# sephiroce/srf

Measured on AMD Instinct MI355X. Metric: acoustic frames/sec through SRF (123-d fbank, 3-iter DR) at 1/2/4/8 MI355X, higher is better.
Workload: dtype fp32; 1 GPU; wsj_c4: SRF L=6 PH=CH=16 DIM=32 LPAD=RPAD=2 DR iter=3, train step (fwd+bwd+allreduce+Adam); utterances_per_gpu=28, frames_per_utterance=800, global_batch=28, parallelism=dp1, launch=hipgraph (fwd+CTC+bwd)

## Files before the change

### srf_amd/csrc/cnnfe.hip

```cpp
#include <algorithm>
#include <cmath>
#include <cstdlib>

#include "srf_common.h"
#include "srf_reduce.h"
#include "srf_rng.h"
#include "../../include/srf.h"

namespace {

constexpr int C = 64;
constexpr float kBnEps = 1e-3f;
constexpr float kBnMomentum = 0.99f;

struct Dims {
  int B, T, Fin;
  int T1, F1, T2, F2;
  int pt1, pf1, pt2, pf2;
};

inline int same_out(int n) { return (n + 1) / 2; }
inline int same_pad_before(int n) {
  const int out = same_out(n);
  const int total = std::max((out - 1) * 2 + 3 - n, 0);
  return total / 2;
}

Dims make_dims(int B, int T, int Fin) {
  Dims d;
  d.B = B; d.T = T; d.Fin = Fin;
  d.T1 = same_out(T); d.F1 = same_out(Fin);
  d.T2 = same_out(d.T1); d.F2 = same_out(d.F1);
  d.pt1 = same_pad_before(T); d.pf1 = same_pad_before(Fin);
  d.pt2 = same_pad_before(d.T1); d.pf2 = same_pad_before(d.F1);
  return d;
}

__device__ __forceinline__ int ceil_div_len(int len, int div) { return (len + div - 1) / div; }

__device__ __forceinline__ void chan_merge(float& n, float& mean, float& m2, float nb, float meanb, float m2b) {
  if (nb == 0.f) return;
  const float nn = n + nb;
  const float delta = meanb - mean;
  mean += delta * (nb / nn);
  m2 += m2b + delta * delta * (n * nb / nn);
  n = nn;
}

constexpr int kPackW2Threads = 2 * C * 64;
__device__ __forceinline__ void pack_w2_f16_body(int idx, const float* __restrict__ ka, const float* __restrict__ kb,
                                                 _Float16* __restrict__ wp2, float* __restrict__ wsc);
__device__ __forceinline__ void pack_w2t_f16_body(int idx, const float* __restrict__ ka, const float* __restrict__ kb,
                                                  _Float16* __restrict__ wq2h, float* __restrict__ wdsc);
constexpr int kPackW2tF16Threads = C * 64;

constexpr int kRows1 = 4;

struct Tile1 {
  int b, t1_0, fpad;
};

__device__ __forceinline__ Tile1 stage_rows1(const float* __restrict__ feats, const Dims& d, float* win) {
  const int tiles_per_b = (d.T1 + kRows1 - 1) / kRows1;
  Tile1 tl;
  tl.b = blockIdx.x / tiles_per_b;
  tl.t1_0 = (blockIdx.x - tl.b * tiles_per_b) * kRows1;
  tl.fpad = d.Fin + 2;
  const int nrows = 2 * kRows1 + 1;
  const int t_base = 2 * tl.t1_0 - d.pt1;
  for (int k = threadIdx.x; k < nrows * tl.fpad; k += blockDim.x) {
    const int r = k / tl.fpad, col = k - r * tl.fpad;
    const int t = t_base + r, f = col - 1;
    const bool ok = t >= 0 && t < d.T && f >= 0 && f < d.Fin;
    const float v = feats[((size_t)tl.b * d.T + min(max(t, 0), d.T - 1)) * d.Fin + min(max(f, 0), d.Fin - 1)];
    win[k] = ok ? v : 0.f;
  }
  __syncthreads();
  return tl;
}

__device__ __forceinline__ void window9_lds(const float* win, const Tile1& tl, const Dims& d, int w, int f1,
                                            float (&x)[9]) {
#pragma unroll
  for (int dt = 0; dt < 3; ++dt)
#pragma unroll
    for (int df = 0; df < 3; ++df) x[dt * 3 + df] = win[(2 * w + dt) * tl.fpad + 2 * f1 - d.pf1 + df + 1];
}

__global__ __launch_bounds__(256) void conv1_fwd_kernel(
    const float* __restrict__ feats, const int* __restrict__ inp_len, Dims d, const float* __restrict__ ka,
    const float* __restrict__ ba, const float* __restrict__ kb, const float* __restrict__ bb, int training,
    float drop_p, unsigned long long seed, const unsigned long long* __restrict__ seed_src, float* __restrict__ y1, unsigned char* __restrict__ sel1,
    float* __restrict__ part, int nconv, const float* __restrict__ pk_a, const float* __restrict__ pk_b,
    _Float16* __restrict__ wp2, float* __restrict__ wsc, float* __restrict__ ymax) {
  if ((int)blockIdx.x >= nconv) {
    const int idx = (blockIdx.x - nconv) * blockDim.x + threadIdx.x;
    if (idx < kPackW2Threads) pack_w2_f16_body(idx, pk_a, pk_b, wp2, wsc);
    return;
  }
  seed = srf_step_seed(seed, seed_src);
  extern __shared__ __attribute__((aligned(16))) float win[];
  __shared__ float sh[3][kRows1][C];
  const int c = threadIdx.x & (C - 1);
  const int w = __builtin_amdgcn_readfirstlane(threadIdx.x >> 6);
  float wa[9], wb[9];
#pragma unroll
  for (int k = 0; k < 9; ++k) {
    wa[k] = ka[k * C + c];
    wb[k] = kb[k * C + c];
  }
  const float bia = ba[c], bib = bb[c];
  const float keep_scale = 1.f / (1.f - drop_p);
  const bool drop = training && drop_p > 0.f;
  const Tile1 tl = stage_rows1(feats, d, win);
  const int t1 = tl.t1_0 + w;
  float n = 0.f, s1 = 0.f, s2 = 0.f, ym = 0.f;
  const float K = 0.5f * (bia + bib);
  if (t1 < d.T1) {
    const bool live = t1 < ceil_div_len(inp_len[tl.b], 2);
    const int pbase = (tl.b * d.T1 + t1) * d.F1;
#pragma unroll 2
    for (int f1 = 0; f1 < d.F1; ++f1) {
      float x[9];
      window9_lds(win, tl, d, w, f1, x);
      float a = bia, bv = bib;
#pragma unroll
      for (int k = 0; k < 9; ++k) {
        a += x[k] * wa[k];
        bv += x[k] * wb[k];
      }
      const int o = (pbase + f1) * C + c;
      if (drop) {
        bool ka, kb;
        srf_keep2(seed, kStreamConv0a, o, drop_p, ka, kb);
        a *= ka ? keep_scale : 0.f;
        bv *= kb ? keep_scale : 0.f;
      }
      const bool sl = a >= bv;
      const float y = live ? (sl ? a : bv) : 0.f;
      y1[o] = y;
      sel1[o] = sl ? 1 : 0;
      ym = fmaxf(ym, fabsf(y));
      n += 1.f;
      s1 += y - K;
      s2 += (y - K) * (y - K);
    }
  }
  float mean = n > 0.f ? K + s1 / n : 0.f;
  float m2 = n > 0.f ? fmaxf(s2 - s1 * s1 / n, 0.f) : 0.f;
  sh[0][w][c] = n; sh[1][w][c] = mean; sh[2][w][c] = m2;
#pragma unroll
  for (int o = 32; o >= 1; o >>= 1) ym = fmaxf(ym, __shfl_xor(ym, o, 64));
  __shared__ float smax[kRows1];
  if (c == 0) smax[w] = ym;
  __syncthreads();
  if (w == 0) {
    if (c == 0) {
      float m = smax[0];
      for (int r = 1; r < kRows1; ++r) m = fmaxf(m, smax[r]);
      ymax[blockIdx.x] = m;
    }
    for (int r = 1; r < kRows1; ++r) chan_merge(n, mean, m2, sh[0][r][c], sh[1][r][c], sh[2][r][c]);
    part[((size_t)blockIdx.x * 3 + 0) * C + c] = n;
    part[((size_t)blockIdx.x * 3 + 1) * C + c] = mean;
    part[((size_t)blockIdx.x * 3 + 2) * C + c] = m2;
  }
}

__global__ __launch_bounds__(256) void bn_merge_kernel(const float* __restrict__ part, int nparts, int per,
                                                       float* __restrict__ out) {
  __shared__ float sh[3][4][C];
  const int c = threadIdx.x & (C - 1), r = threadIdx.x >> 6;
  const int k0 = blockIdx.x * per, k1 = min(nparts, k0 + per);
  float n = 0.f, mu = 0.f, m2 = 0.f;
  for (int k = k0 + r; k < k1; k += 4)
    chan_merge(n, mu, m2, part[((size_t)k * 3 + 0) * C + c], part[((size_t)k * 3 + 1) * C + c],
               part[((size_t)k * 3 + 2) * C + c]);
  sh[0][r][c] = n; sh[1][r][c] = mu; sh[2][r][c] = m2;
  __syncthreads();
  if (r != 0) return;
  for (int q = 1; q < 4; ++q) chan_merge(n, mu, m2, sh[0][q][c], sh[1][q][c], sh[2][q][c]);
  out[((size_t)blockIdx.x * 3 + 0) * C + c] = n;
  out[((size_t)blockIdx.x * 3 + 1) * C + c] = mu;
  out[((size_t)blockIdx.x * 3 + 2) * C + c] = m2;
}

__global__ __launch_bounds__(1024) void bn_finalize_kernel(const float* __restrict__ part, int nparts,
                                                           const float* __restrict__ gamma,
                                                           const float* __restrict__ beta,
                                                           float* __restrict__ mmean, float* __restrict__ mvar,
                                                           int training, float* __restrict__ stats,
                                                           const float* __restrict__ ymax, int nymax) {
  __shared__ float sh[3][16][C];
  __shared__ float ysh[16], ab[2][C];
  const int c = threadIdx.x & (C - 1), r = threadIdx.x >> 6;
  if (ymax != nullptr) {
    float m = 0.f;
    for (int k = threadIdx.x; k < nymax; k += 1024) m = fmaxf(m, ymax[k]);
#pragma unroll
    for (int o = 32; o >= 1; o >>= 1) m = fmaxf(m, __shfl_xor(m, o, 64));
    if (c == 0) ysh[r] = m;
  }
  float n = 0.f, mu = 0.f, m2 = 0.f;
  if (training)
#pragma unroll 8
    for (int k = r; k < nparts; k += 16)
      chan_merge(n, mu, m2, part[((size_t)k * 3 + 0) * C + c], part[((size_t)k * 3 + 1) * C + c],
                 part[((size_t)k * 3 + 2) * C + c]);
  sh[0][r][c] = n; sh[1][r][c] = mu; sh[2][r][c] = m2;
  __syncthreads();
  if (r == 0) {
    float mean, var;
    if (training) {
      for (int q = 1; q < 16; ++q) chan_merge(n, mu, m2, sh[0][q][c], sh[1][q][c], sh[2][q][c]);
      mean = mu;
      var = m2 / n;
      mmean[c] = mmean[c] * kBnMomentum + mean * (1.f - kBnMomentum);
      mvar[c] = mvar[c] * kBnMomentum + (n > 1.f ? var * n / (n - 1.f) : var) * (1.f - kBnMomentum);
    } else {
      mean = mmean[c];
      var = mvar[c];
    }
    const float rstd = 1.f / sqrtf(var + kBnEps);
    const float scale = gamma[c] * rstd;
    const float shift = beta[c] - mean * scale;
    stats[0 * C + c] = mean;
    stats[1 * C + c] = rstd;
    stats[2 * C + c] = scale;
    stats[3 * C + c] = shift;
    ab[0][c] = fabsf(scale);
    ab[1][c] = fabsf(shift);
  }
  if (ymax == nullptr) return;
  __syncthreads();
  if (threadIdx.x == 0) {
    float y = ysh[0], sa = 0.f, sb = 0.f;
    for (int q = 1; q < 16; ++q) y = fmaxf(y, ysh[q]);
    for (int q = 0; q < C; ++q) {
      sa = fmaxf(sa, ab[0][q]);
      sb = fmaxf(sb, ab[1][q]);
    }
    const int e = srf_split_exp(sa * y + sb);
    stats[4 * C + 0] = srf_exp2i(e);
    stats[4 * C + 1] = srf_exp2i(-e);
  }
}


__device__ __forceinline__ void split2h8(const float (&v)[8], h8& p1, h8& p2, float sc = 1.f) {
#pragma unroll
  for (int k = 0; k < 8; ++k) {
    _Float16 h1, h2;
    srf_split2h(v[k] * sc, h1, h2);
    p1[k] = h1;
    p2[k] = h2;
  }
}
__device__ __forceinline__ f16v mfma3h(const h8& a1, const h8& a2, const h8& b1, const h8& b2, f16v c) {
  c = mfma32h(a2, b1, c);
  c = mfma32h(a1, b2, c);
  return mfma32h(a1, b1, c);
}

__device__ __forceinline__ void pack_w2_f16_body(int idx, const float* __restrict__ ka, const float* __restrict__ kb,
                                                 _Float16* __restrict__ wp2, float* __restrict__ wsc) {
  const int n = idx >> 6, cin = idx & 63;
  const float* k = n < C ? ka : kb;
  const int co = n % C;
  float v[9], m = 0.f;
#pragma unroll
  for (int tap = 0; tap < 9; ++tap) {
    v[tap] = k[((size_t)tap * C + cin) * C + co];
    m = fmaxf(m, fabsf(v[tap]));
  }
#pragma unroll
  for (int o = 32; o >= 1; o >>= 1) m = fmaxf(m, __shfl_xor(m, o, 64));
  const int e = srf_split_exp(m);
  const float sc = srf_exp2i(e);
  const size_t plane = (size_t)9 * 2 * C * C;
#pragma unroll
  for (int tap = 0; tap < 9; ++tap) {
    _Float16 h1, h2;
    srf_split2h(v[tap] * sc, h1, h2);
    const size_t o = ((size_t)tap * 2 * C + n) * C + cin;
    wp2[o] = h1;
    wp2[plane + o] = h2;
  }
  if (cin == 0) wsc[n] = srf_exp2i(-e);
}

constexpr int kC2BStride = 24;
constexpr int kC2Waves = 4;
constexpr int kC2Px = 32 * kC2Waves;
constexpr int kC2BLoads = 2 * 2 * C * 2 / (64 * kC2Waves);

__global__ __launch_bounds__(64 * kC2Waves) __attribute__((amdgpu_waves_per_eu(2))) void conv2_fwd32_kernel(
    const float* __restrict__ y1, const float* __restrict__ stats1, const int* __restrict__ inp_len, Dims d,
    const _Float16* __restrict__ wp2, const float* __restrict__ wsc, const float* __restrict__ ba,
    const float* __restrict__ bb, int training, float drop_p, unsigned long long seed,
    const unsigned long long* __restrict__ seed_src, float* __restrict__ y2, unsigned char* __restrict__ sel2,
    float* __restrict__ part) {
  seed = srf_step_seed(seed, seed_src);
  __shared__ __attribute__((aligned(16))) _Float16 Bs[2][2][2 * C * kC2BStride];
  __shared__ __attribute__((aligned(16))) float ss[2][C];
  __shared__ float red[3][kC2Waves][2 * 32];
  const int tid = threadIdx.x;
  const int lane = tid & 63, wv = tid >> 6;
  const int r = lane & 31, h = lane >> 5;
  const int P2 = d.B * d.T2 * d.F2;
  const int p0 = blockIdx.x * kC2Px;
  const size_t plane = (size_t)9 * 2 * C * C;
  if (tid < 2 * C) ss[tid >> 6][tid & 63] = stats1[(2 + (tid >> 6)) * C + (tid & 63)] * stats1[4 * C];

  const int pa = p0 + 32 * wv + r;
  const bool alive = pa < P2;
  const int pc = min(pa, P2 - 1);
  const int af2 = pc % d.F2, at2 = (pc / d.F2) % d.T2, ab = pc / (d.F2 * d.T2);
  const int alen1 = ceil_div_len(inp_len[ab], 2);

  auto load_b = [&](int kk, h8 (&bv)[kC2BLoads]) {
    const int tap = kk >> 2, kb = kk & 3;
#pragma unroll
    for (int q = 0; q < kC2BLoads; ++q) {
      const int idx = q * 64 * kC2Waves + tid;
      const int pl = idx >> 8, rem = idx & 255, n = rem >> 1, half = rem & 1;
      bv[q] = *reinterpret_cast<const h8*>(wp2 + pl * plane + ((size_t)tap * 2 * C + n) * C + 16 * kb + 8 * half);
    }
  };
  auto store_b = [&](int buf, const h8 (&bv)[kC2BLoads]) {
#pragma unroll
    for (int q = 0; q < kC2BLoads; ++q) {
      const int idx = q * 64 * kC2Waves + tid;
      const int pl = idx >> 8, rem = idx & 255, n = rem >> 1, half = rem & 1;
      *reinterpret_cast<h8*>(&Bs[buf][pl][n * kC2BStride + 8 * half]) = bv[q];
    }
  };
  auto load_a = [&](int kk, f4 (&av)[2], bool& ok) {
    const int tap = kk >> 2, kb = kk & 3;
    const int dt = tap / 3, df = tap - dt * 3;
    const int t1 = 2 * at2 - d.pt2 + dt, f1 = 2 * af2 - d.pf2 + df;
    ok = alive && t1 >= 0 && t1 < d.T1 && f1 >= 0 && f1 < d.F1 && t1 < alen1;
    const int t1c = min(max(t1, 0), d.T1 - 1), f1c = min(max(f1, 0), d.F1 - 1);
    const float* src = y1 + (((size_t)ab * d.T1 + t1c) * d.F1 + f1c) * C + 16 * kb + 8 * h;
    av[0] = *reinterpret_cast<const f4*>(src);
    av[1] = *reinterpret_cast<const f4*>(src + 4);
  };

  f16v acc[4];
#pragma unroll
  for (int nt = 0; nt < 4; ++nt) acc[nt] = f16v{};
  auto compute = [&](int kk, int buf, const f4 (&av)[2], bool aok) {
    h8 a1, a2;
    {
      const int c0 = 16 * (kk & 3) + 8 * h;
      float v[8];
#pragma unroll
      for (int q = 0; q < 8; ++q) {
        const float x = q < 4 ? av[0][q] : av[1][q - 4];
        v[q] = aok ? x * ss[0][c0 + q] + ss[1][c0 + q] : 0.f;
      }
      split2h8(v, a1, a2);
    }
#pragma unroll
    for (int nt = 0; nt < 4; ++nt) {
      const int nrow = (nt >> 1) * C + 32 * (nt & 1) + r;
      const h8 b1 = *reinterpret_cast<const h8*>(&Bs[buf][0][nrow * kC2BStride + 8 * h]);
      const h8 b2 = *reinterpret_cast<const h8*>(&Bs[buf][1][nrow * kC2BStride + 8 * h]);
      acc[nt] = mfma3h(a1, a2, b1, b2, acc[nt]);
    }
  };
  h8 bvA[kC2BLoads], bvB[kC2BLoads];
  f4 avA[2], avB[2], avC[2];
  bool okA, okB, okC;
  load_b(0, bvA);
  load_a(0, avA, okA);
  load_b(1, bvB);
  load_a(1, avB, okB);
  store_b(0, bvA);
  __syncthreads();
  for (int kk = 0; kk < 36; kk += 2) {
    {
      const f4 a0[2] = {avA[0], avA[1]};
      const bool ok0 = okA;
      if (kk + 2 < 36) {
        load_b(kk + 2, bvA);
        load_a(kk + 2, avA, okA);
      }
      compute(kk, 0, a0, ok0);
      store_b(1, bvB);
      __syncthreads();
    }
    {
      const f4 a1v[2] = {avB[0], avB[1]};
      const bool ok1 = okB;
      if (kk + 3 < 36) {
        load_b(kk + 3, bvB);
        load_a(kk + 3, avB, okB);
      }
      compute(kk + 1, 1, a1v, ok1);
      if (kk + 2 < 36) store_b(0, bvA);
      __syncthreads();
    }
  }
  (void)avC;
  (void)okC;

  const float keep_scale = 1.f / (1.f - drop_p);
  const float inv_b = stats1[4 * C + 1];
#pragma unroll
  for (int g = 0; g < 2; ++g) {
    const int c = 32 * g + r;
    const float bia = ba[c], bib = bb[c];
    const float sca = wsc[c] * inv_b, scb = wsc[C + c] * inv_b;
    float n = 0.f, mean = 0.f, m2 = 0.f;
#pragma unroll
    for (int q = 0; q < 4; ++q)
#pragma unroll
// ... 429 lines not shown
__device__ __forceinline__ ws4 lds_tr16(const _Float16* p) {
  return __builtin_amdgcn_ds_read_tr16_b64_v4i16(
      (__attribute__((address_space(3))) ws4*)(reinterpret_cast<uintptr_t>(p)));
}

__global__ __launch_bounds__(256) __attribute__((amdgpu_waves_per_eu(2))) void conv2_wgrad32_kernel(
    const float* __restrict__ y1, const float* __restrict__ stats1, const int* __restrict__ inp_len,
    const _Float16* __restrict__ gsT, int P2p, Dims d, WgDiv dv, int nsplit, int split_len, float* __restrict__ part,
    const float* __restrict__ gmax, int ngmax) {
  __shared__ __attribute__((aligned(16))) _Float16 As[2][2][kW2Chunk * kW2AStride];
  const float out_sc = stats1[4 * C + 1] * srf_exp2i(-gab_exp(gmax, ngmax));
  const int tid = threadIdx.x, lane = tid & 63, wv = tid >> 6;
  const int r = lane & 31, h = lane >> 5;
  const int xcd = blockIdx.x & 7, loc = blockIdx.x >> 3;
  const int tap = loc % 9, sp = xcd + 8 * (loc / 9);
  const int dt = tap / 3, df = tap - dt * 3;
  const int P2 = d.B * d.T2 * d.F2;
  const int pbeg = sp * split_len, pend = min(P2, pbeg + split_len);
  const int px = tid >> 3, oc = tid & 7;
  float scale[8], shift[8];
  const float bsc = stats1[4 * C];
#pragma unroll
  for (int k = 0; k < 8; ++k) {
    scale[k] = stats1[2 * C + 8 * oc + k] * bsc;
    shift[k] = stats1[3 * C + 8 * oc + k] * bsc;
  }
  f4 xv[2];
  bool xok = false;
  auto gather = [&](int pc0) {
    const int p = pc0 + px;
    const unsigned pcl = (unsigned)min(p, P2 - 1);
    const unsigned r1 = fdiv(pcl, dv.f2);
    const int f2 = (int)(pcl - r1 * d.F2);
    const unsigned bq = fdiv(r1, dv.t2);
    const int t2 = (int)(r1 - bq * d.T2), b = (int)bq;
    const int t1 = 2 * t2 - d.pt2 + dt, f1 = 2 * f2 - d.pf2 + df;
    xok = p < pend && t1 >= 0 && t1 < d.T1 && f1 >= 0 && f1 < d.F1 && t1 < ceil_div_len(inp_len[b], 2);
    const int t1c = min(max(t1, 0), d.T1 - 1), f1c = min(max(f1, 0), d.F1 - 1);
    const float* src = y1 + (((size_t)b * d.T1 + t1c) * d.F1 + f1c) * C + 8 * oc;
    xv[0] = *reinterpret_cast<const f4*>(src);
    xv[1] = *reinterpret_cast<const f4*>(src + 4);
  };
  auto put = [&](int buf) {
    float v[8];
#pragma unroll
    for (int k = 0; k < 8; ++k) v[k] = xok ? (k < 4 ? xv[0][k] : xv[1][k - 4]) * scale[k] + shift[k] : 0.f;
    const int o = px * kW2AStride + 8 * oc;
    h8 p1, p2;
    split2h8(v, p1, p2);
    *reinterpret_cast<h8*>(&As[buf][0][o]) = p1;
    *reinterpret_cast<h8*>(&As[buf][1][o]) = p2;
  };
  const int gg = lane >> 4, qq = (lane >> 2) & 3, pp = lane & 3;
  const int a_off = (8 * (gg >> 1) + qq) * kW2AStride + 16 * (gg & 1) + 4 * pp;
  auto read_a = [&](const _Float16* img, int kb, int mt) {
    const _Float16* base = img + a_off + 16 * kb * kW2AStride + 32 * mt;
    const ws4 lo = lds_tr16(base), hi = lds_tr16(base + 4 * kW2AStride);
    return __builtin_bit_cast(h8, __builtin_shufflevector(lo, hi, 0, 1, 2, 3, 4, 5, 6, 7));
  };
  const size_t bplane = (size_t)2 * C * P2p;
  const _Float16* brow = gsT + (size_t)(32 * wv + r) * P2p + 8 * h;
  h8 bc[2][2], bn[2][2];
  auto load_bf = [&](int pc0, h8 (&bf)[2][2]) {
#pragma unroll
    for (int kb = 0; kb < 2; ++kb)
#pragma unroll
      for (int pl = 0; pl < 2; ++pl) bf[kb][pl] = *reinterpret_cast<const h8*>(brow + pl * bplane + pc0 + 16 * kb);
  };

  f16v acc[2];
  acc[0] = f16v{};
  acc[1] = f16v{};
  const int nch = (pend - pbeg + kW2Chunk - 1) / kW2Chunk;
  if (nch > 0) {
    gather(pbeg);
    load_bf(pbeg, bc);
    put(0);
  }
  __syncthreads();
  for (int ch = 0; ch < nch; ++ch) {
    const bool more = ch + 1 < nch;
    const int buf = ch & 1;
    if (more) {
      gather(pbeg + (ch + 1) * kW2Chunk);
      load_bf(pbeg + (ch + 1) * kW2Chunk, bn);
    }
#pragma unroll
    for (int kb = 0; kb < 2; ++kb)
#pragma unroll
      for (int mt = 0; mt < 2; ++mt) {
        const h8 a1 = read_a(As[buf][0], kb, mt);
        const h8 a2 = read_a(As[buf][1], kb, mt);
        acc[mt] = mfma3h(a1, a2, bc[kb][0], bc[kb][1], acc[mt]);
      }
    if (more) {
      put(buf ^ 1);
#pragma unroll
      for (int kb = 0; kb < 2; ++kb)
#pragma unroll
        for (int pl = 0; pl < 2; ++pl) bc[kb][pl] = bn[kb][pl];
    }
    __syncthreads();
  }
  float* dst = part + ((size_t)sp * 9 + tap) * C * 2 * C + 32 * wv + r;
#pragma unroll
  for (int mt = 0; mt < 2; ++mt)
#pragma unroll
    for (int q = 0; q < 4; ++q)
#pragma unroll
      for (int v = 0; v < 4; ++v) dst[(size_t)(32 * mt + 8 * q + 4 * h + v) * 2 * C] = acc[mt][4 * q + v] * out_sc;
}

__global__ void conv2_wgrad_reduce_kernel(const float* __restrict__ part, int nsplit, float* __restrict__ gka,
                                          float* __restrict__ gkb) {
  const int idx = blockIdx.x * blockDim.x + threadIdx.x;
  if (idx >= 9 * C * 2 * C) return;
  float s = 0.f;
#pragma unroll 8
  for (int k = 0; k < nsplit; ++k) s += part[(size_t)k * 9 * C * 2 * C + idx];
  const int n = idx % (2 * C);
  const int tc = idx / (2 * C);
  if (n < C)
    gka[(size_t)tc * C + n] = s;
  else
    gkb[(size_t)tc * C + n - C] = s;
}

#ifndef SRF_CONV2_WGRAD_ROWS
#define SRF_CONV2_WGRAD_ROWS 1
#endif

constexpr int kWrRanges = 256;
constexpr int kWrCh = 32;
constexpr int kWrSub = 33 * kWrCh;
constexpr int kWrSlot = 4 * kWrSub;
constexpr int kWrBStride = 160;
constexpr int kWrBPlane = 32 * kWrBStride;

__global__ __launch_bounds__(256) __attribute__((amdgpu_waves_per_eu(2))) void conv2_wgrad_rows_kernel(
    const float* __restrict__ y1, const float* __restrict__ stats1, const int* __restrict__ inp_len,
    const float* __restrict__ g_ab, Dims d, int rows_per, float* __restrict__ part, const float* __restrict__ gmax,
    int ngmax) {
  __shared__ __attribute__((aligned(16))) _Float16 As[4 * kWrSlot];
  __shared__ __attribute__((aligned(16))) _Float16 Bs[2 * kWrBPlane];
  const int tid = threadIdx.x, lane = tid & 63, wv = tid >> 6;
  const int r = lane & 31, h = lane >> 5;
  const int hc = (blockIdx.x >> 3) & 1, rg = (blockIdx.x & 7) + 8 * (blockIdx.x >> 4);
  const int R = d.B * d.T2;
  const int rbeg = (int)min((long long)R, (long long)rg * rows_per), rend = min(R, rbeg + rows_per);
  for (int k = tid; k < 4 * kWrSlot / 8; k += 256) *reinterpret_cast<h8*>(&As[8 * k]) = h8{};
  for (int k = tid; k < 2 * kWrBPlane / 8; k += 256) *reinterpret_cast<h8*>(&Bs[8 * k]) = h8{};
  const int ea = gab_exp(gmax, ngmax);
  const float sa = srf_exp2i(ea);
  const float out_sc = stats1[4 * C + 1] * srf_exp2i(-ea);
  __syncthreads();

  const int ac = tid >> 2, aoc = tid & 3;
  const int af1 = ac - d.pf2;
  const bool acol_ok = af1 >= 0 && af1 < d.F1;
  const int af1c = min(max(af1, 0), d.F1 - 1);
  const int a_lds = (ac & 1) * 2 * kWrSub + (ac >> 1) * kWrCh + 8 * aoc;
  const int bpx = tid >> 4, bo = tid & 15;
  float scale[8], shift[8];
  const float bsc = stats1[4 * C];
#pragma unroll
  for (int k = 0; k < 8; ++k) {
    scale[k] = stats1[2 * C + 32 * hc + 8 * aoc + k] * bsc;
    shift[k] = stats1[3 * C + 32 * hc + 8 * aoc + k] * bsc;
  }
  f4 xv[3][2], gv[2][2];
  bool xok[3] = {false, false, false};
  auto load_row = [&](int b, int t2, bool fresh) {
    const int alen1 = ceil_div_len(inp_len[b], 2);
#pragma unroll
    for (int dt = 0; dt < 3; ++dt) {
      if (dt == 0 && !fresh) continue;
      const int t1 = 2 * t2 - d.pt2 + dt;
      xok[dt] = acol_ok && t1 >= 0 && t1 < d.T1 && t1 < alen1;
      const int t1c = min(max(t1, 0), d.T1 - 1);
      const float* src = y1 + (((size_t)b * d.T1 + t1c) * d.F1 + af1c) * C + 32 * hc + 8 * aoc;
      xv[dt][0] = *reinterpret_cast<const f4*>(src);
      xv[dt][1] = *reinterpret_cast<const f4*>(src + 4);
    }
#pragma unroll
    for (int u = 0; u < 2; ++u) {
      const int pxc = min(bpx + 16 * u, d.F2 - 1);
      const float* src = g_ab + (((size_t)b * d.T2 + t2) * d.F2 + pxc) * 2 * C + 8 * bo;
      gv[u][0] = *reinterpret_cast<const f4*>(src);
      gv[u][1] = *reinterpret_cast<const f4*>(src + 4);
    }
  };
  auto put_row = [&](int t2, bool fresh) {
#pragma unroll
    for (int dt = 0; dt < 3; ++dt) {
      if (dt == 0 && !fresh) continue;
      h8 p1, p2;
#pragma unroll
      for (int k = 0; k < 8; ++k) {
        const float v = xok[dt] ? (k < 4 ? xv[dt][0][k] : xv[dt][1][k - 4]) * scale[k] + shift[k] : 0.f;
        _Float16 h1, h2;
        srf_split2h(v, h1, h2);
        p1[k] = h1;
        p2[k] = h2;
      }
      _Float16* dst = As + ((2 * t2 + dt) & 3) * kWrSlot + a_lds;
      *reinterpret_cast<h8*>(dst) = p1;
      *reinterpret_cast<h8*>(dst + kWrSub) = p2;
    }
#pragma unroll
    for (int u = 0; u < 2; ++u) {
      const int px = bpx + 16 * u;
      const bool ok = px < d.F2;
      h8 p1, p2;
#pragma unroll
      for (int k = 0; k < 8; ++k) {
        const float v = ok ? (k < 4 ? gv[u][0][k] : gv[u][1][k - 4]) * sa : 0.f;
        _Float16 h1, h2;
        srf_split2h(v, h1, h2);
        p1[k] = h1;
        p2[k] = h2;
      }
      _Float16* dst = Bs + px * kWrBStride + 8 * bo;
      *reinterpret_cast<h8*>(dst) = p1;
      *reinterpret_cast<h8*>(dst + kWrBPlane) = p2;
    }
  };
  const int gg = lane >> 4, qq = (lane >> 2) & 3, pp = lane & 3;
  const int a_off = (8 * (gg >> 1) + qq) * kWrCh + 16 * (gg & 1) + 4 * pp;
  const int b_off = (8 * (gg >> 1) + qq) * kWrBStride + 32 * wv + 16 * (gg & 1) + 4 * pp;
  auto tr8 = [&](const _Float16* base, int stride) {
    const ws4 lo = lds_tr16(base), hi = lds_tr16(base + 4 * stride);
    return __builtin_bit_cast(h8, __builtin_shufflevector(lo, hi, 0, 1, 2, 3, 4, 5, 6, 7));
  };
  f16v acc[9];
#pragma unroll
  for (int tap = 0; tap < 9; ++tap) acc[tap] = f16v{};
  auto compute = [&](int t2) {
#pragma unroll
    for (int kb = 0; kb < 2; ++kb) {
      const h8 b1 = tr8(Bs + b_off + 16 * kb * kWrBStride, kWrBStride);
      const h8 b2 = tr8(Bs + kWrBPlane + b_off + 16 * kb * kWrBStride, kWrBStride);
#pragma unroll
      for (int tap = 0; tap < 9; ++tap) {
        const int dt = tap / 3, df = tap - dt * 3;
        const _Float16* img =
            As + ((2 * t2 + dt) & 3) * kWrSlot + (df & 1) * 2 * kWrSub + ((df >> 1) + 16 * kb) * kWrCh + a_off;
        const h8 a1 = tr8(img, kWrCh);
        const h8 a2 = tr8(img + kWrSub, kWrCh);
        acc[tap] = mfma3h(a1, a2, b1, b2, acc[tap]);
      }
    }
  };

  int b = rbeg / d.T2, t2 = rbeg - b * d.T2;
  if (rbeg < rend) {
    load_row(b, t2, true);
    put_row(t2, true);
  }
  __syncthreads();
  for (int row = rbeg; row < rend; ++row) {
    const bool more = row + 1 < rend;
    const bool nfresh = t2 + 1 == d.T2;
    const int nb = nfresh ? b + 1 : b, nt2 = nfresh ? 0 : t2 + 1;
    if (more) load_row(nb, nt2, nfresh);
    compute(t2);
    __syncthreads();
    if (more) put_row(nt2, nfresh);
    __syncthreads();
    b = nb;
    t2 = nt2;
  }
  float* dst = part + ((size_t)rg * 9 * C + 32 * hc) * 2 * C + 32 * wv + r;
#pragma unroll
  for (int tap = 0; tap < 9; ++tap)
#pragma unroll
    for (int q = 0; q < 4; ++q)
#pragma unroll
      for (int v = 0; v < 4; ++v)
        dst[((size_t)tap * C + 8 * q + 4 * h + v) * 2 * C] = acc[tap][4 * q + v] * out_sc;
}

__global__ __launch_bounds__(256) void conv2_wgrad_reduce_rows_kernel(const float* __restrict__ part,
                                                                      float* __restrict__ gka,
                                                                      float* __restrict__ gkb) {
  static_assert(kWrRanges == 256 && (9 * C * 2 * C) % 128 == 0, "eight groups of 32 slabs");
  __shared__ f4 sums[8][32];
  const int j = threadIdx.x & 31, g = threadIdx.x >> 5;
  const size_t idx = (size_t)blockIdx.x * 128 + 4 * j;
  const float* src = part + (size_t)g * 9 * C * 2 * C + idx;
  f4 s = {0.f, 0.f, 0.f, 0.f};
#pragma unroll 8
  for (int k = 0; k < 32; ++k) s += *reinterpret_cast<const f4*>(src + (size_t)8 * k * 9 * C * 2 * C);
  sums[g][j] = s;
  __syncthreads();
  if (g != 0) return;
  for (int k = 1; k < 8; ++k) s += sums[k][j];
  const int n = (int)(idx % (2 * C));
  const size_t tc = idx / (2 * C);
  float* dst = n < C ? gka + tc * C + n : gkb + tc * C + n - C;
#pragma unroll
  for (int k = 0; k < 4; ++k) dst[k] = s[k];
}

__global__ __launch_bounds__(256) void conv1_bwd_kernel(
    const float* __restrict__ feats, const int* __restrict__ inp_len, Dims d, const float* __restrict__ g_x1,
    const float* __restrict__ y1, const unsigned char* __restrict__ sel1, const float* __restrict__ stats1,
    const float* __restrict__ gamma1, const float* __restrict__ bnsum1, float drop_p, unsigned long long seed, const unsigned long long* __restrict__ seed_src,
    float* __restrict__ part) {
  seed = srf_step_seed(seed, seed_src);
  extern __shared__ __attribute__((aligned(16))) float win[];
  __shared__ float sh[kRows1][20][C];
  const int c = threadIdx.x & (C - 1);
  const int w = __builtin_amdgcn_readfirstlane(threadIdx.x >> 6);
  const int P = d.B * d.T1 * d.F1;
  const float mean = stats1[c], rstd = stats1[C + c], gam = gamma1[c];
  const float sdy_n = bnsum1[c] / (float)P, sdyxh_n = bnsum1[C + c] / (float)P;
  const float keep_scale = 1.f / (1.f - drop_p);
  float acc[20];
#pragma unroll
  for (int j = 0; j < 20; ++j) acc[j] = 0.f;
  const Tile1 tl = stage_rows1(feats, d, win);
  const int t1 = tl.t1_0 + w;
  if (t1 < d.T1) {
    const float mask = t1 < ceil_div_len(inp_len[tl.b], 2) ? 1.f : 0.f;
    const int pbase = (tl.b * d.T1 + t1) * d.F1;
    constexpr int FB = 8;
    for (int f0 = 0; f0 < d.F1; f0 += FB) {
      float gxv[FB], yv[FB];
      unsigned char sv[FB];
#pragma unroll
      for (int u = 0; u < FB; ++u) {
        const int o = (pbase + min(f0 + u, d.F1 - 1)) * C + c;
        gxv[u] = g_x1[o];
        yv[u] = y1[o];
        sv[u] = sel1[o];
      }
#pragma unroll
      for (int u = 0; u < FB; ++u) {
        const int f1 = f0 + u;
        if (f1 >= d.F1) break;
        const int o = (pbase + f1) * C + c;
        const float gy = bn_bwd_elem(gxv[u], yv[u], mask, mean, rstd, gam, sdy_n, sdyxh_n);
        const bool sl = sv[u] != 0;
        float ga = sl ? gy : 0.f, gb = sl ? 0.f : gy;
        if (drop_p > 0.f) {
          bool ka, kb;
          srf_keep2(seed, kStreamConv0a, o, drop_p, ka, kb);
          ga *= ka ? keep_scale : 0.f;
          gb *= kb ? keep_scale : 0.f;
        }
        float x[9];
        window9_lds(win, tl, d, w, f1, x);
        acc[18] += ga;
        acc[19] += gb;
#pragma unroll
        for (int k = 0; k < 9; ++k) {
          acc[k] += x[k] * ga;
          acc[9 + k] += x[k] * gb;
        }
      }
    }
  }
#pragma unroll
  for (int j = 0; j < 20; ++j) sh[w][j][c] = acc[j];
  __syncthreads();
  for (int j = w; j < 20; j += kRows1) {
    float v = 0.f;
#pragma unroll
    for (int r = 0; r < kRows1; ++r) v += sh[r][j][c];
    part[((size_t)blockIdx.x * 20 + j) * C + c] = v;
  }
}

inline int conv1_blocks(const Dims& d) { return d.B * ((d.T1 + kRows1 - 1) / kRows1); }
inline size_t conv1_lds(const Dims& d) { return (size_t)(2 * kRows1 + 1) * (d.Fin + 2) * sizeof(float); }

struct FwdSaved {
  float *y1, *y2, *stats1, *stats2;
  unsigned char *sel1, *sel2;
  size_t bytes;
};

struct Bump {
  size_t off = 0;
  size_t take(size_t bytes) {
    const size_t o = off;
    off += srf::align_up(bytes, 256);
    return o;
  }
};

FwdSaved saved_layout(const Dims& d, void* base) {
  const size_t P1 = (size_t)d.B * d.T1 * d.F1, P2 = (size_t)d.B * d.T2 * d.F2;
  Bump bp;
  const size_t oy1 = bp.take(P1 * C * 4), oy2 = bp.take(P2 * C * 4), os1 = bp.take(5 * C * 4),
               os2 = bp.take(5 * C * 4), osel1 = bp.take(P1 * C), osel2 = bp.take(P2 * C);
  char* b = static_cast<char*>(base);
  FwdSaved s;
  s.y1 = (float*)(b + oy1);
  s.y2 = (float*)(b + oy2);
  s.stats1 = (float*)(b + os1);
  s.stats2 = (float*)(b + os2);
  s.sel1 = (unsigned char*)(b + osel1);
  s.sel2 = (unsigned char*)(b + osel2);
  s.bytes = bp.off;
  return s;
}

constexpr int kBnMerge = 32;

int bn_finalize(const float* part, int nparts, float* merged, const float* gamma, const float* beta, float* mmean,
                float* mvar, int training, float* stats, hipStream_t st, const float* ymax = nullptr,
                int nymax = 0) {
  const int per = (nparts + kBnMerge - 1) / kBnMerge;
  hipLaunchKernelGGL(bn_merge_kernel, dim3(kBnMerge), dim3(256), 0, st, part, nparts, per, merged);
  SRF_LAUNCH_CHECK("bn_merge");
  hipLaunchKernelGGL(bn_finalize_kernel, dim3(1), dim3(1024), 0, st, merged, kBnMerge, gamma, beta, mmean, mvar,
                     training, stats, ymax, nymax);
  SRF_LAUNCH_CHECK("bn_finalize");
  return SRF_OK;
}

struct FwdWs {
  float *part1, *part2, *merged;
  _Float16* wp2;
  float* wsc;
  float* ymax;
  size_t bytes;
};

FwdWs fwd_ws_layout(const Dims& d, void* base) {
  const size_t P2 = (size_t)d.B * d.T2 * d.F2;
  const size_t nb2 = (P2 + 63) / 64;
  Bump bp;
  const size_t op1 = bp.take((size_t)conv1_blocks(d) * 3 * C * 4), op2 = bp.take(nb2 * 3 * C * 4),
               omg = bp.take((size_t)kBnMerge * 3 * C * 4), owp2 = bp.take((size_t)2 * 9 * 2 * C * C * 2),
               owsc = bp.take((size_t)2 * C * 4), oym = bp.take((size_t)conv1_blocks(d) * 4);
  char* b = static_cast<char*>(base);
  FwdWs w;
  w.wp2 = (_Float16*)(b + owp2);
  w.wsc = (float*)(b + owsc);
  w.ymax = (float*)(b + oym);
  w.merged = (float*)(b + omg);
  w.part1 = (float*)(b + op1);
  w.part2 = (float*)(b + op2);
  w.bytes = bp.off;
  return w;
}

int check_dims(int B, int T, int Fin, int nfilt) {
  SRF_REQUIRE(B > 0 && T > 0 && Fin > 0, "bad CNN-FE shape B=%d T=%d F=%d", B, T, Fin);
  SRF_REQUIRE(nfilt == C, "model-conv-filter-num must be %d (got %d)", C, nfilt);
  return SRF_OK;
}

}

extern "C" {

int srf_cnnfe_out_dims(int T, int feat_dim, int* T2, int* F2) {
  SRF_REQUIRE(T > 0 && feat_dim > 0 && T2 && F2, "bad arguments");
  Dims d = make_dims(1, T, feat_dim);
  *T2 = d.T2;
  *F2 = d.F2;
  return SRF_OK;
}

size_t srf_cnnfe_saved_bytes(int B, int T, int feat_dim, int nfilt) {
  (void)nfilt;
  return saved_layout(make_dims(B, T, feat_dim), nullptr).bytes;
}

size_t srf_cnnfe_fwd_workspace(int B, int T, int feat_dim, int nfilt) {
  (void)nfilt;
  return fwd_ws_layout(make_dims(B, T, feat_dim), nullptr).bytes;
}

int srf_cnnfe_fwd(const float* feats, const int* inp_len, int B, int T, int feat_dim, int nfilt,
                  const float* k0a, const float* b0a, const float* k0b, const float* b0b, const float* gamma0,
                  const float* beta0, const float* k1a, const float* b1a, const float* k1b, const float* b1b,
                  const float* gamma1, const float* beta1, float* mmean0, float* mvar0, float* mmean1, float* mvar1,
                  int training, float drop_p, unsigned long long seed, float* out, void* saved, size_t saved_bytes,
                  void* workspace, size_t workspace_bytes, void* stream) {
  int rc = check_dims(B, T, feat_dim, nfilt);
  if (rc) return rc;
  SRF_REQUIRE(feats && inp_len && k0a && b0a && k0b && b0b && gamma0 && beta0 && k1a && b1a && k1b && b1b &&
                  gamma1 && beta1 && mmean0 && mvar0 && mmean1 && mvar1 && out && saved && workspace,
              "null pointer argument");
  SRF_REQUIRE(drop_p >= 0.f && drop_p < 1.f, "dropout rate %f out of [0,1)", drop_p);
  const Dims d = make_dims(B, T, feat_dim);
  FwdSaved sv = saved_layout(d, saved);
  FwdWs w = fwd_ws_layout(d, workspace);
  if (saved_bytes < sv.bytes || workspace_bytes < w.bytes) {
    srf::set_error("CNN-FE buffers too small (saved %zu < %zu or workspace %zu < %zu)", saved_bytes, sv.bytes,
                   workspace_bytes, w.bytes);
    return SRF_EWORKSPACE;
  }
  hipStream_t st = static_cast<hipStream_t>(stream);
  const size_t P2 = (size_t)d.B * d.T2 * d.F2;
  const int nb2 = (int)((P2 + 63) / 64);
  int nparts2 = nb2;
  const int npack = (kPackW2Threads + 64 * kRows1 - 1) / (64 * kRows1);
  hipLaunchKernelGGL(conv1_fwd_kernel, dim3(conv1_blocks(d) + npack), dim3(64 * kRows1), conv1_lds(d), st, feats,
                     inp_len, d, k0a, b0a, k0b, b0b, training, drop_p, seed, srf::seed_source(), sv.y1, sv.sel1,
                     w.part1, conv1_blocks(d), k1a, k1b, w.wp2, w.wsc, w.ymax);
  SRF_LAUNCH_CHECK("conv1_fwd");
  if ((rc = bn_finalize(w.part1, conv1_blocks(d), w.merged, gamma0, beta0, mmean0, mvar0, training, sv.stats1, st,
                        w.ymax, conv1_blocks(d))))
    return rc;
  SRF_LAUNCH_CHECK("bn_finalize(1)");
  {
    const int nb32 = (int)((P2 + kC2Px - 1) / kC2Px);
    hipLaunchKernelGGL(conv2_fwd32_kernel, dim3(nb32), dim3(64 * kC2Waves), 0, st, sv.y1, sv.stats1, inp_len, d,
                       w.wp2, w.wsc, b1a, b1b, training, drop_p, seed, srf::seed_source(), sv.y2, sv.sel2,
                       w.part2);
    SRF_LAUNCH_CHECK("conv2_fwd32");
    nparts2 = nb32;
  }
  if ((rc = bn_finalize(w.part2, nparts2, w.merged, gamma1, beta1, mmean1, mvar1, training, sv.stats2, st)))
    return rc;
  SRF_LAUNCH_CHECK("bn_finalize(2)");
  hipLaunchKernelGGL(bn_apply_kernel, dim3(1024), dim3(256), 0, st, sv.y2, sv.stats2, inp_len, d.B, d.T2, d.F2, 4,
                     out);
  SRF_LAUNCH_CHECK("bn_apply");
  return SRF_OK;
}

}

namespace {
struct BwdWs2 {
  float *bnpart, *bnsum2, *bnsum1, *g_ab, *biaspart, *g_x1, *wpart, *c1part, *c1sum, *scratch;
  _Float16* wq2h;
  _Float16* gsT;
  float* gmax;
  float* wdsc;
  int P2p;
  size_t bytes;
};

constexpr int kBnBlocks = 1024;
constexpr int kWgrad32SplitsMax = 128;
constexpr int kWgrad32Splits = 56;
inline bool wgrad_by_rows(const Dims& d) { return SRF_CONV2_WGRAD_ROWS && d.F2 <= 32; }

BwdWs2 bwd_ws_layout(const Dims& d, void* base) {
  const size_t P1 = (size_t)d.B * d.T1 * d.F1, P2 = (size_t)d.B * d.T2 * d.F2;
  Bump bp;
  const size_t obp = bp.take((size_t)kBnBlocks * 2 * C * 4), os2 = bp.take(2 * C * 4), os1 = bp.take(2 * C * 4),
               oab = bp.take(P2 * 2 * C * 4), obias = bp.take((size_t)kBnBlocks * 2 * C * 4),
               ogx = bp.take(P1 * C * 4), owq = bp.take((size_t)2 * 9 * C * 2 * C * 2),
               owp = bp.take((size_t)std::max(kWgrad32SplitsMax, kWrRanges) * 9 * C * 2 * C * 4),
               oc1 = bp.take((size_t)conv1_blocks(d) * 20 * C * 4), oc1s = bp.take(20 * C * 4),
               oscr = bp.take(srf::colsum_scratch_floats(std::max(conv1_blocks(d), kBnBlocks), 20 * C) * 4);
  const int P2p = (int)((P2 + kTpPx - 1) / kTpPx * kTpPx);
  const size_t ogs = bp.take(wgrad_by_rows(d) ? 0 : (size_t)2 * 2 * C * P2p * 2);
  const size_t ogm = bp.take((size_t)kBnBlocks * 4), ods = bp.take((size_t)C * 4);
  char* b = static_cast<char*>(base);
  BwdWs2 w;
  w.bnpart = (float*)(b + obp);
  w.bnsum2 = (float*)(b + os2);
  w.bnsum1 = (float*)(b + os1);
  w.g_ab = (float*)(b + oab);
  w.biaspart = (float*)(b + obias);
  w.g_x1 = (float*)(b + ogx);
  w.wq2h = (_Float16*)(b + owq);
  w.wpart = (float*)(b + owp);
  w.c1part = (float*)(b + oc1);
  w.c1sum = (float*)(b + oc1s);
  w.scratch = (float*)(b + oscr);
  w.gsT = (_Float16*)(b + ogs);
  w.gmax = (float*)(b + ogm);
  w.wdsc = (float*)(b + ods);
  w.P2p = P2p;
  w.bytes = bp.off;
  return w;
}

}

extern "C" {

size_t srf_cnnfe_bwd_workspace(int B, int T, int feat_dim, int nfilt) {
  (void)nfilt;
  return bwd_ws_layout(make_dims(B, T, feat_dim), nullptr).bytes;
}

int srf_cnnfe_bwd(const float* feats, const int* inp_len, int B, int T, int feat_dim, int nfilt, const float* gamma0,
                  const float* k1a, const float* k1b, const float* gamma1, float drop_p, unsigned long long seed,
                  const void* saved, const float* g_out, float* g_k0a, float* g_b0a, float* g_k0b, float* g_b0b,
                  float* g_gamma0, float* g_beta0, float* g_k1a, float* g_b1a, float* g_k1b, float* g_b1b,
                  float* g_gamma1, float* g_beta1, void* workspace, size_t workspace_bytes, void* stream) {
  return srf_cnnfe_bwd_parts(SRF_CNNFE_BWD_ALL, feats, inp_len, B, T, feat_dim, nfilt, gamma0, k1a, k1b, gamma1, drop_p,
                             seed, saved, g_out, g_k0a, g_b0a, g_k0b, g_b0b, g_gamma0, g_beta0, g_k1a, g_b1a, g_k1b,
                             g_b1b, g_gamma1, g_beta1, workspace, workspace_bytes, stream);
}

int srf_cnnfe_bwd_parts(int parts, const float* feats, const int* inp_len, int B, int T, int feat_dim, int nfilt,
                        const float* gamma0, const float* k1a, const float* k1b, const float* gamma1, float drop_p,
                        unsigned long long seed, const void* saved, const float* g_out, float* g_k0a, float* g_b0a,
                        float* g_k0b, float* g_b0b, float* g_gamma0, float* g_beta0, float* g_k1a, float* g_b1a,
                        float* g_k1b, float* g_b1b, float* g_gamma1, float* g_beta1, void* workspace,
                        size_t workspace_bytes, void* stream) {
  SRF_REQUIRE(parts > 0 && (parts & ~SRF_CNNFE_BWD_ALL) == 0, "CNN-FE backward: bad parts mask %d", parts);
  int rc = check_dims(B, T, feat_dim, nfilt);
  if (rc) return rc;
  SRF_REQUIRE(feats && inp_len && gamma0 && k1a && k1b && gamma1 && saved && g_out && g_k0a && g_b0a && g_k0b &&
                  g_b0b && g_gamma0 && g_beta0 && g_k1a && g_b1a && g_k1b && g_b1b && g_gamma1 && g_beta1 &&
                  workspace,
              "null pointer argument");
  SRF_REQUIRE(((uintptr_t)g_out & 15) == 0 && ((uintptr_t)saved & 255) == 0 && ((uintptr_t)workspace & 255) == 0,
              "CNN-FE backward: g_out must be 16-byte and saved / workspace 256-byte aligned");
  const Dims d = make_dims(B, T, feat_dim);
  FwdSaved sv = saved_layout(d, const_cast<void*>(saved));
  BwdWs2 w = bwd_ws_layout(d, workspace);
  if (workspace_bytes < w.bytes) {
    srf::set_error("CNN-FE backward workspace too small: %zu < %zu", workspace_bytes, w.bytes);
    return SRF_EWORKSPACE;
  }
  hipStream_t st = static_cast<hipStream_t>(stream);
  const int P2 = d.B * d.T2 * d.F2;
  if (parts & SRF_CNNFE_BWD_PREP) {
    hipLaunchKernelGGL(bn_bwd_reduce_kernel, dim3(kBnBlocks), dim3(256), 0, st, g_out, sv.y2, sv.stats2, inp_len,
                       d.B, d.T2, d.F2, 4, w.bnpart);
    SRF_LAUNCH_CHECK("bn_bwd_reduce(2)");
    if ((rc = srf::colsum(w.bnpart, kBnBlocks, 2 * C, w.bnsum2, w.scratch, st,
                          srf::ColSplit{{g_beta1, g_gamma1, nullptr, nullptr}, {C, C, 0, 0}})))
      return rc;
    const int npack = (kPackW2tF16Threads + 255) / 256;
    hipLaunchKernelGGL(conv2_bwd_prep_kernel, dim3(kBnBlocks + npack), dim3(256), 0, st, g_out, sv.y2, sv.sel2,
                       sv.stats2, gamma1, w.bnsum2, inp_len, d, drop_p, seed, srf::seed_source(), w.g_ab,
                       w.biaspart, kBnBlocks, k1a, k1b, w.wq2h, w.wdsc, w.gmax);
    SRF_LAUNCH_CHECK("conv2_bwd_prep");
    if ((rc = srf::colsum(w.biaspart, kBnBlocks, 2 * C, nullptr, w.scratch, st,
                          srf::ColSplit{{g_b1a, g_b1b, nullptr, nullptr}, {C, C, 0, 0}})))
      return rc;
  }
  if (parts & SRF_CNNFE_BWD_DATA) {
    DgCls cls{};
    for (int c = 0; c < 4; ++c) {
      const int qt = c >> 1, qf = c & 1;
      const int Pc = d.B * ((d.T1 - qt + 1) / 2) * ((d.F1 - qf + 1) / 2);
      cls.boff[c + 1] = cls.boff[c] + (Pc + kD2Px - 1) / kD2Px;
    }
    hipLaunchKernelGGL(conv2_dgrad32_kernel, dim3(cls.boff[4]), dim3(64 * kD2Waves), 0, st, w.g_ab,
                       (const _Float16*)w.wq2h, d, cls, w.g_x1, (const float*)w.gmax, kBnBlocks,
                       (const float*)w.wdsc);
    SRF_LAUNCH_CHECK("conv2_dgrad32");
  }
  const WgDiv dv{make_fastdiv(d.F2), make_fastdiv(d.T2)};
  const int nsplit = kWgrad32Splits;
  if ((parts & SRF_CNNFE_BWD_WGRAD) && wgrad_by_rows(d)) {
    const int rows_per = (d.B * d.T2 + kWrRanges - 1) / kWrRanges;
    hipLaunchKernelGGL(conv2_wgrad_rows_kernel, dim3(2 * kWrRanges), dim3(256), 0, st, sv.y1, sv.stats1, inp_len,
                       (const float*)w.g_ab, d, rows_per, w.wpart, (const float*)w.gmax, kBnBlocks);
    SRF_LAUNCH_CHECK("conv2_wgrad_rows");
    hipLaunchKernelGGL(conv2_wgrad_reduce_rows_kernel, dim3(9 * C * 2 * C / 128), dim3(256), 0, st, w.wpart, g_k1a,
                       g_k1b);
    SRF_LAUNCH_CHECK("conv2_wgrad_reduce_rows");
  } else if (parts & SRF_CNNFE_BWD_WGRAD) {
    static_assert(kW2Chunk == kWgChunk, "wgrad splits are whole chunks");
    const int split_len = ((P2 + nsplit - 1) / nsplit + kWgChunk - 1) / kWgChunk * kWgChunk;
    hipLaunchKernelGGL(gab_split_t_kernel, dim3(w.P2p / kTpPx), dim3(256), 0, st, w.g_ab, P2, w.P2p, w.gsT,
                       (const float*)w.gmax, kBnBlocks);
    SRF_LAUNCH_CHECK("gab_split_t");
    hipLaunchKernelGGL(conv2_wgrad32_kernel, dim3(9 * nsplit), dim3(256), 0, st, sv.y1, sv.stats1, inp_len,
                       (const _Float16*)w.gsT, w.P2p, d, dv, nsplit, split_len, w.wpart, (const float*)w.gmax,
                       kBnBlocks);
    SRF_LAUNCH_CHECK("conv2_wgrad32");
    hipLaunchKernelGGL(conv2_wgrad_reduce_kernel, dim3((9 * C * 2 * C + 255) / 256), dim3(256), 0, st, w.wpart,
                       nsplit, g_k1a, g_k1b);
    SRF_LAUNCH_CHECK("conv2_wgrad_reduce");
  }
  if (!(parts & SRF_CNNFE_BWD_DATA)) return SRF_OK;
  hipLaunchKernelGGL(bn_bwd_reduce_kernel, dim3(kBnBlocks), dim3(256), 0, st, w.g_x1, sv.y1, sv.stats1, inp_len, d.B,
                     d.T1, d.F1, 2, w.bnpart);
  SRF_LAUNCH_CHECK("bn_bwd_reduce(1)");
  if ((rc = srf::colsum(w.bnpart, kBnBlocks, 2 * C, w.bnsum1, w.scratch, st, srf::ColSplit{{g_beta0, g_gamma0, nullptr, nullptr}, {C, C, 0, 0}})))
    return rc;
  hipLaunchKernelGGL(conv1_bwd_kernel, dim3(conv1_blocks(d)), dim3(64 * kRows1), conv1_lds(d), st, feats, inp_len, d, w.g_x1, sv.y1,
                     sv.sel1, sv.stats1, gamma0, w.bnsum1, drop_p, seed, srf::seed_source(), w.c1part);
  SRF_LAUNCH_CHECK("conv1_bwd");
  if ((rc = srf::colsum(w.c1part, conv1_blocks(d), 20 * C, nullptr, w.scratch, st,
                        srf::ColSplit{{g_k0a, g_k0b, g_b0a, g_b0b, nullptr, nullptr}, {9 * C, 9 * C, C, C, 0, 0}})))
    return rc;
  return SRF_OK;
}

}
```

Before: 3.330 million frames/s.

## Fuse BN backward reduction into conv1 backward via algebraic decomposition

Removes the separate BN-backward reduction pass and its colsum over g_x1/y1 before conv1 backward. The BN input-gradient formula is split into three accumulated moments (x*k*g, x*k, x*k*xhat) plus the sums of g and g*xhat, so the whole thing runs in one pass; a small finalize kernel combines them afterwards. The kernel also becomes persistent with a grid-stride loop over tiles, double-buffers the per-channel loads, and caps the partial rows to shrink the follow-up colsum. In exchange it uses more registers (three times the accumulators), and recombining the moments may lose some fp32 precision.

```diff
diff --git a/srf_amd/csrc/cnnfe.hip b/srf_amd/csrc/cnnfe.hip
--- a/srf_amd/csrc/cnnfe.hip
+++ b/srf_amd/csrc/cnnfe.hip
@@ -60,12 +60,17 @@
   int b, t1_0, fpad;
 };
 
-__device__ __forceinline__ Tile1 stage_rows1(const float* __restrict__ feats, const Dims& d, float* win) {
+__device__ __forceinline__ Tile1 tile1_of(const Dims& d, int tile) {
   const int tiles_per_b = (d.T1 + kRows1 - 1) / kRows1;
   Tile1 tl;
-  tl.b = blockIdx.x / tiles_per_b;
-  tl.t1_0 = (blockIdx.x - tl.b * tiles_per_b) * kRows1;
+  tl.b = tile / tiles_per_b;
+  tl.t1_0 = (tile - tl.b * tiles_per_b) * kRows1;
   tl.fpad = d.Fin + 2;
+  return tl;
+}
+
+__device__ __forceinline__ Tile1 stage_rows1(const float* __restrict__ feats, const Dims& d, float* win, int tile) {
+  const Tile1 tl = tile1_of(d, tile);
   const int nrows = 2 * kRows1 + 1;
   const int t_base = 2 * tl.t1_0 - d.pt1;
   for (int k = threadIdx.x; k < nrows * tl.fpad; k += blockDim.x) {
@@ -112,7 +117,7 @@
   const float bia = ba[c], bib = bb[c];
   const float keep_scale = 1.f / (1.f - drop_p);
   const bool drop = training && drop_p > 0.f;
-  const Tile1 tl = stage_rows1(feats, d, win);
+  const Tile1 tl = stage_rows1(feats, d, win, blockIdx.x);
   const int t1 = tl.t1_0 + w;
   float n = 0.f, s1 = 0.f, s2 = 0.f, ym = 0.f;
   const float K = 0.5f * (bia + bib);
@@ -1148,6 +1153,151 @@
   for (int k = 0; k < 4; ++k) dst[k] = s[k];
 }
 
+#ifndef SRF_CONV1_BWD_FUSED
+#define SRF_CONV1_BWD_FUSED 1
+#endif
+
+#if SRF_CONV1_BWD_FUSED
+constexpr int kC1Cols = 62;
+constexpr int kC1Pass = kC1Cols / 2;
+
+__global__ __launch_bounds__(256) void conv1_bwd_kernel(
+    const float* __restrict__ feats, const int* __restrict__ inp_len, Dims d, int ntiles,
+    const float* __restrict__ g_x1, const float* __restrict__ y1, const unsigned char* __restrict__ sel1,
+    const float* __restrict__ stats1, float drop_p, unsigned long long seed,
+    const unsigned long long* __restrict__ seed_src, float* __restrict__ part) {
+  seed = srf_step_seed(seed, seed_src);
+  extern __shared__ __attribute__((aligned(16))) float win[];
+  __shared__ float sh[kRows1][kC1Pass][C];
+  const int c = threadIdx.x & (C - 1);
+  const int w = __builtin_amdgcn_readfirstlane(threadIdx.x >> 6);
+  const float mean = stats1[c], rstd = stats1[C + c];
+  const float keep_scale = 1.f / (1.f - drop_p);
+  f2 acc[3][10];
+#pragma unroll
+  for (int q = 0; q < 3; ++q)
+#pragma unroll
+    for (int k = 0; k < 10; ++k) acc[q][k] = f2{0.f, 0.f};
+  float sg = 0.f, sgxh = 0.f;
+  constexpr int FB = 8;
+  struct Batch {
+    float g[FB], y[FB];
+    unsigned char s[FB];
+  };
+  auto load_batch = [&](int pbase, int f0, Batch& bt) {
+#pragma unroll
+    for (int u = 0; u < FB; ++u) {
+      const int o = (pbase + min(f0 + u, d.F1 - 1)) * C + c;
+      bt.g[u] = g_x1[o];
+      bt.y[u] = y1[o];
+      bt.s[u] = sel1[o];
+    }
+  };
+  auto compute_batch = [&](const Tile1& tl, int pbase, int f0, const Batch& bt) {
+#pragma unroll
+    for (int u = 0; u < FB; ++u) {
+      const int f1 = f0 + u;
+      if (f1 >= d.F1) break;
+      const int o = (pbase + f1) * C + c;
+      const float g = bt.g[u];
+      const float xh = (bt.y[u] - mean) * rstd;
+      sg += g;
+      sgxh += g * xh;
+      const bool sl = bt.s[u] != 0;
+      float ka_s = sl ? 1.f : 0.f, kb_s = sl ? 0.f : 1.f;
+      if (drop_p > 0.f) {
+        bool ka, kb;
+        srf_keep2(seed, kStreamConv0a, o, drop_p, ka, kb);
+        ka_s *= ka ? keep_scale : 0.f;
+        kb_s *= kb ? keep_scale : 0.f;
+      }
+      const f2 k2 = f2{ka_s, kb_s};
+      const f2 w1 = k2 * g, w3 = k2 * xh;
+      float x[9];
+      window9_lds(win, tl, d, w, f1, x);
+      acc[0][9] += w1;
+      acc[1][9] += k2;
+      acc[2][9] += w3;
+#pragma unroll
+      for (int k = 0; k < 9; ++k) {
+        acc[0][k] = x[k] * w1 + acc[0][k];
+        acc[1][k] = x[k] * k2 + acc[1][k];
+        acc[2][k] = x[k] * w3 + acc[2][k];
+      }
+    }
+  };
+  for (int tile = blockIdx.x; tile < ntiles; tile += gridDim.x) {
+    const Tile1 tl = tile1_of(d, tile);
+    const int t1 = tl.t1_0 + w;
+    const bool live = t1 < d.T1 && t1 < ceil_div_len(inp_len[tl.b], 2);
+    const int pbase = (tl.b * d.T1 + min(t1, d.T1 - 1)) * d.F1;
+    Batch ba, bb;
+    if (live) load_batch(pbase, 0, ba);
+    if (tile != (int)blockIdx.x) __syncthreads();
+    stage_rows1(feats, d, win, tile);
+    if (!live) continue;
+    for (int f0 = 0; f0 < d.F1; f0 += 2 * FB) {
+      const bool more = f0 + FB < d.F1;
+      if (more) load_batch(pbase, f0 + FB, bb);
+      compute_batch(tl, pbase, f0, ba);
+      if (!more) break;
+      if (f0 + 2 * FB < d.F1) load_batch(pbase, f0 + 2 * FB, ba);
+      compute_batch(tl, pbase, f0 + FB, bb);
+    }
+  }
+  float col[kC1Cols];
+#pragma unroll
+  for (int q = 0; q < 3; ++q) {
+#pragma unroll
+    for (int k = 0; k < 9; ++k) {
+      col[20 * q + k] = acc[q][k].x;
+      col[20 * q + 9 + k] = acc[q][k].y;
+    }
+    col[20 * q + 18] = acc[q][9].x;
+    col[20 * q + 19] = acc[q][9].y;
+  }
+  col[60] = sg;
+  col[61] = sgxh;
+#pragma unroll
+  for (int ps = 0; ps < 2; ++ps) {
+    if (ps) __syncthreads();
+#pragma unroll
+    for (int j = 0; j < kC1Pass; ++j) sh[w][j][c] = col[ps * kC1Pass + j];
+    __syncthreads();
+    for (int j = w; j < kC1Pass; j += kRows1) {
+      float v = 0.f;
+#pragma unroll
+      for (int r = 0; r < kRows1; ++r) v += sh[r][j][c];
+      part[((size_t)blockIdx.x * kC1Cols + ps * kC1Pass + j) * C + c] = v;
+    }
+  }
+}
+
+__global__ __launch_bounds__(256) void conv1_bwd_finalize_kernel(
+    const float* __restrict__ sums, const float* __restrict__ stats1, const float* __restrict__ gamma1, int P,
+    float* __restrict__ g_ka, float* __restrict__ g_kb, float* __restrict__ g_ba, float* __restrict__ g_bb,
+    float* __restrict__ g_beta, float* __restrict__ g_gamma) {
+  const int idx = blockIdx.x * blockDim.x + threadIdx.x;
+  if (idx >= 20 * C) return;
+  const int j = idx / C, c = idx - j * C;
+  const float sdy = sums[60 * C + c], sdyxh = sums[61 * C + c];
+  const float s1 = sdy / (float)P, s2 = sdyxh / (float)P;
+  const float t1 = sums[(0 * 20 + j) * C + c], t2 = sums[(1 * 20 + j) * C + c], t3 = sums[(2 * 20 + j) * C + c];
+  const float v = gamma1[c] * stats1[C + c] * (t1 - s1 * t2 - s2 * t3);
+  if (j < 9)
+    g_ka[j * C + c] = v;
+  else if (j < 18)
+    g_kb[(j - 9) * C + c] = v;
+  else if (j == 18)
+    g_ba[c] = v;
+  else
+    g_bb[c] = v;
+  if (j == 0) {
+    g_beta[c] = sdy;
+    g_gamma[c] = sdyxh;
+  }
+}
+#else
 __global__ __launch_bounds__(256) void conv1_bwd_kernel(
     const float* __restrict__ feats, const int* __restrict__ inp_len, Dims d, const float* __restrict__ g_x1,
     const float* __restrict__ y1, const unsigned char* __restrict__ sel1, const float* __restrict__ stats1,
@@ -1165,7 +1315,7 @@
   float acc[20];
 #pragma unroll
   for (int j = 0; j < 20; ++j) acc[j] = 0.f;
-  const Tile1 tl = stage_rows1(feats, d, win);
+  const Tile1 tl = stage_rows1(feats, d, win, blockIdx.x);
   const int t1 = tl.t1_0 + w;
   if (t1 < d.T1) {
     const float mask = t1 < ceil_div_len(inp_len[tl.b], 2) ? 1.f : 0.f;
@@ -1217,8 +1367,15 @@
     part[((size_t)blockIdx.x * 20 + j) * C + c] = v;
   }
 }
+#endif
 
 inline int conv1_blocks(const Dims& d) { return d.B * ((d.T1 + kRows1 - 1) / kRows1); }
+#if SRF_CONV1_BWD_FUSED
+inline int conv1_bwd_rows(const Dims& d) {
+  const int fit = std::min(conv1_blocks(d) * 20 / kC1Cols, 1024);
+  return fit >= 256 ? fit / 256 * 256 : fit;
+}
+#endif
 inline size_t conv1_lds(const Dims& d) { return (size_t)(2 * kRows1 + 1) * (d.Fin + 2) * sizeof(float); }
 
 struct FwdSaved {
@@ -1519,6 +1676,21 @@
     SRF_LAUNCH_CHECK("conv2_wgrad_reduce");
   }
   if (!(parts & SRF_CNNFE_BWD_DATA)) return SRF_OK;
+#if SRF_CONV1_BWD_FUSED
+  static_assert((size_t)2 * kC1Cols * C <= (size_t)kBnBlocks * 2 * C, "a partial row and the sums fit bnpart");
+  const int fit = conv1_bwd_rows(d);
+  const int nrows = std::max(fit, 1);
+  float* c1part = fit > 0 ? w.c1part : w.bnpart;
+  float* c1sums = w.bnpart + (size_t)kC1Cols * C;
+  hipLaunchKernelGGL(conv1_bwd_kernel, dim3(nrows), dim3(64 * kRows1), conv1_lds(d), st, feats, inp_len, d,
+                     conv1_blocks(d), w.g_x1, sv.y1, sv.sel1, sv.stats1, drop_p, seed, srf::seed_source(), c1part);
+  SRF_LAUNCH_CHECK("conv1_bwd");
+  if ((rc = srf::colsum(c1part, nrows, kC1Cols * C, c1sums, w.scratch, st))) return rc;
+  hipLaunchKernelGGL(conv1_bwd_finalize_kernel, dim3((20 * C + 255) / 256), dim3(256), 0, st, (const float*)c1sums,
+                     sv.stats1, gamma0, d.B * d.T1 * d.F1, g_k0a, g_k0b, g_b0a, g_b0b, g_beta0, g_gamma0);
+  SRF_LAUNCH_CHECK("conv1_bwd_finalize");
+  return SRF_OK;
+#else
   hipLaunchKernelGGL(bn_bwd_reduce_kernel, dim3(kBnBlocks), dim3(256), 0, st, w.g_x1, sv.y1, sv.stats1, inp_len, d.B,
                      d.T1, d.F1, 2, w.bnpart);
   SRF_LAUNCH_CHECK("bn_bwd_reduce(1)");
@@ -1531,6 +1703,7 @@
                         srf::ColSplit{{g_k0a, g_k0b, g_b0a, g_b0b, nullptr, nullptr}, {9 * C, 9 * C, C, C, 0, 0}})))
     return rc;
   return SRF_OK;
-}
-
-}
+#endif
+}
+
+}
```

Result: no change. 3.346 million frames/s (median of 6 runs) (+0.5%).
